# huggingface/open-muse

Measured on AMD Instinct MI355X. Metric: images/sec/node (MaskGit train step, 256^2, bs=64/GPU), higher is better.
Workload: dtype bf16 (transformer GEMM/attention operands; f32 accumulate, residual, norms, loss) + bf16x3 tokenizer (f32 activations, f32-class products as 3 bf16 MFMAs); parity of this mode was not measured in this run (a --full run measures it); 1 GPU; MaskGit train step: MaskGitVQGAN f16-256 encode (bf16x3) + cosine mask + MaskGitTransformer config B (configs/imagenet.yaml: hidden 768, 24 layers, 16 heads, vocab 2048, seq 257) fwd+bwd (bf16 MFMA, f32 accum/residual) + AdamW; global_batch=64, per_gpu_batch=64, resolution=256, seq_len=257, parallelism=dp1, vqgan_dtype=bf16x3, random_init=True, wgrad_stream=True

## Files before the change

### open-muse_amd/csrc/embed.hip

```cpp
#include <cstring>
#include <rocprim/device/device_radix_sort.hpp>
#include "common.h"
#include "../../include/muse_hip.h"

namespace emb {
constexpr int SEG = 64;

__global__ void prep_kernel(const int64_t* __restrict__ ids, unsigned* __restrict__ keys, unsigned* __restrict__ vals, int ntok, int vocab) {
  const int t = blockIdx.x * blockDim.x + threadIdx.x;
  if (t < ntok) {
    const int64_t id = ids[t];
    keys[t] = (id >= 0 && id < vocab) ? (unsigned)id : (unsigned)vocab;
    vals[t] = (unsigned)t;
  }
}

__global__ __launch_bounds__(1024) void table_kernel(const unsigned* __restrict__ keys, int ntok, int vocab, int* __restrict__ start,
                                                     int* __restrict__ segfirst) {
  __shared__ int wsum[16];
  __shared__ int carry_s;
  for (int v = threadIdx.x; v <= vocab; v += 1024) {
    int lo = 0, hi = ntok;
    while (lo < hi) { const int mid = (lo + hi) >> 1; if (keys[mid] < (unsigned)v) lo = mid + 1; else hi = mid; }
    start[v] = lo;
  }
  if (threadIdx.x == 0) carry_s = 0;
  __syncthreads();
  const int lane = threadIdx.x & 63, wave = threadIdx.x >> 6;
  for (int base = 0; base <= vocab; base += 1024) {
    const int v = base + threadIdx.x;
    int n = 0;
    if (v < vocab) n = (start[v + 1] - start[v] + SEG - 1) / SEG;
    int incl = n;
#pragma unroll
    for (int o = 1; o < 64; o <<= 1) { const int y = __shfl_up(incl, o, 64); if (lane >= o) incl += y; }
    if (lane == 63) wsum[wave] = incl;
    __syncthreads();
    int woff = 0;
    for (int w = 0; w < wave; ++w) woff += wsum[w];
    const int carry = carry_s;
    if (v <= vocab) segfirst[v] = carry + woff + incl - n;
    __syncthreads();
    if (threadIdx.x == 1023) carry_s = carry + woff + incl;
    __syncthreads();
  }
}

__global__ __launch_bounds__(256) void segment_kernel(const unsigned* __restrict__ order, const int* __restrict__ start,
                                                      const int* __restrict__ segfirst, const float* __restrict__ dout,
                                                      float* __restrict__ partial, int hidden, int vocab) {
  const int b = blockIdx.x;
  if (b >= segfirst[vocab]) return;
  int lo = 0, hi = vocab;
  while (hi - lo > 1) { const int mid = (lo + hi) >> 1; if (segfirst[mid] <= b) lo = mid; else hi = mid; }
  const int v = lo;
  const int p0 = start[v] + (b - segfirst[v]) * SEG, p1 = min(start[v + 1], p0 + SEG);
  float acc[16];
#pragma unroll
  for (int j = 0; j < 16; ++j) acc[j] = 0.f;
  const int ncol = (hidden - (int)threadIdx.x + 255) / 256;
  int h = p0;
  for (; h + 4 <= p1; h += 4) {
    const float* s0 = dout + (long)order[h] * hidden;
    const float* s1 = dout + (long)order[h + 1] * hidden;
    const float* s2 = dout + (long)order[h + 2] * hidden;
    const float* s3 = dout + (long)order[h + 3] * hidden;
#pragma unroll
    for (int j = 0; j < 16; ++j) {
      if (j < ncol) {
        const int c = threadIdx.x + j * 256;
        const float a0 = s0[c], a1 = s1[c], a2 = s2[c], a3 = s3[c];
        acc[j] = (((acc[j] + a0) + a1) + a2) + a3;
      }
    }
  }
  for (; h < p1; ++h) {
    const float* src = dout + (long)order[h] * hidden;
#pragma unroll
    for (int j = 0; j < 16; ++j) if (j < ncol) acc[j] += src[threadIdx.x + j * 256];
  }
  float* dst = partial + (long)b * hidden;
#pragma unroll
  for (int j = 0; j < 16; ++j) { const int c = threadIdx.x + j * 256; if (c < hidden) dst[c] = acc[j]; }
}

__global__ __launch_bounds__(256) void row_kernel(const int* __restrict__ segfirst, const float* __restrict__ partial,
                                                  float* __restrict__ dword, int hidden, int accumulate) {
  const int v = blockIdx.x, s0 = segfirst[v], s1 = segfirst[v + 1];
  for (int c = threadIdx.x; c < hidden; c += 256) {
    float s = 0.f;
    for (int k = s0; k < s1; ++k) s += partial[(long)k * hidden + c];
    float* d = dword + (long)v * hidden + c;
    *d = accumulate ? *d + s : s;
  }
}

__global__ void pos_kernel(const float* __restrict__ dout, float* __restrict__ dpos, int batch, int seq, int hidden, int acc) {
  const int s = blockIdx.x;
  for (int c = threadIdx.x; c < hidden; c += blockDim.x) {
    float a = 0.f;
    for (int b = 0; b < batch; ++b) a += dout[((long)b * seq + s) * hidden + c];
    float* d = dpos + (long)s * hidden + c;
    *d = acc ? *d + a : a;
  }
}

static inline size_t al(size_t x) { return (x + 255) & ~(size_t)255; }
struct Layout { size_t keys_in, keys_out, vals_in, vals_out, start, segfirst, partial, temp, temp_bytes, total; int maxseg; };
static inline int key_bits(int vocab) { int b = 1; while ((1 << b) <= vocab) ++b; return b; }
static int layout(int ntok, int hidden, int vocab, Layout& L) {
  size_t tb = 0;
  const hipError_t e = rocprim::radix_sort_pairs((void*)nullptr, tb, (const unsigned*)nullptr, (unsigned*)nullptr, (const unsigned*)nullptr,
                                                 (unsigned*)nullptr, (size_t)ntok, 0u, (unsigned)key_bits(vocab), (hipStream_t)0);
  if (e != hipSuccess) return (int)e;
  L.maxseg = vocab + ntok / SEG + 1;
  size_t o = 0;
  L.keys_in = o; o += al((size_t)ntok * 4);
  L.keys_out = o; o += al((size_t)ntok * 4);
  L.vals_in = o; o += al((size_t)ntok * 4);
  L.vals_out = o; o += al((size_t)ntok * 4);
  L.start = o; o += al((size_t)(vocab + 1) * 4);
  L.segfirst = o; o += al((size_t)(vocab + 1) * 4);
  L.partial = o; o += al((size_t)L.maxseg * hidden * 4);
  L.temp = o; L.temp_bytes = tb; o += al(tb);
  L.total = o;
  return 0;
}
}

extern "C" int64_t muse_embed_bwd2_scratch_bytes(int32_t batch, int32_t seq, int32_t hidden, int32_t vocab) {
  emb::Layout L;
  if (batch <= 0 || seq <= 0) return 0;
  if (emb::layout(batch * seq, hidden, vocab, L)) return -1;
  return (int64_t)L.total;
}

extern "C" int muse_embed_bwd2(const int64_t* ids, const float* dout, float* dword, float* dpos, void* scratch, int64_t scratch_bytes,
                               int32_t batch, int32_t seq, int32_t hidden, int32_t vocab, int32_t accumulate, void* stream) {
  if (hidden > 4096 || vocab <= 0) return MUSE_ERR_UNSUPPORTED;
  const int ntok = batch * seq;
  if (ntok <= 0) return 0;
  emb::Layout L;
  if (int e = emb::layout(ntok, hidden, vocab, L)) return e;
  if ((size_t)scratch_bytes < L.total || (((uintptr_t)scratch) & 255)) return MUSE_ERR_BAD_ARG;
  hipStream_t s = (hipStream_t)stream;
  unsigned char* base = (unsigned char*)scratch;
  unsigned* keys_in = (unsigned*)(base + L.keys_in);
  unsigned* keys_out = (unsigned*)(base + L.keys_out);
  unsigned* vals_in = (unsigned*)(base + L.vals_in);
  unsigned* vals_out = (unsigned*)(base + L.vals_out);
  int* start = (int*)(base + L.start);
  int* segfirst = (int*)(base + L.segfirst);
  float* partial = (float*)(base + L.partial);
  hipLaunchKernelGGL(emb::prep_kernel, dim3((ntok + 255) / 256), dim3(256), 0, s, ids, keys_in, vals_in, ntok, vocab);
  size_t tb = L.temp_bytes;
  const hipError_t e = rocprim::radix_sort_pairs((void*)(base + L.temp), tb, (const unsigned*)keys_in, keys_out, (const unsigned*)vals_in, vals_out,
                                                 (size_t)ntok, 0u, (unsigned)emb::key_bits(vocab), s);
  if (e != hipSuccess) return (int)e;
  hipLaunchKernelGGL(emb::table_kernel, dim3(1), dim3(1024), 0, s, (const unsigned*)keys_out, ntok, vocab, start, segfirst);
  hipLaunchKernelGGL(emb::segment_kernel, dim3(L.maxseg), dim3(256), 0, s, (const unsigned*)vals_out, (const int*)start, (const int*)segfirst,
                     dout, partial, hidden, vocab);
  hipLaunchKernelGGL(emb::row_kernel, dim3(vocab), dim3(256), 0, s, (const int*)segfirst, (const float*)partial, dword, hidden, accumulate);
  hipLaunchKernelGGL(emb::pos_kernel, dim3(seq), dim3(256), 0, s, dout, dpos, batch, seq, hidden, accumulate);
  return (int)hipGetLastError();
}
```

### open-muse_amd/csrc/rowops.hip

```cpp
#include "common.h"
#include "../../include/muse_hip.h"

template <typename TI, typename TO>
__global__ __launch_bounds__(256) void ln_fwd_kernel(const TI* __restrict__ x, const float* __restrict__ w,
                                                     const float* __restrict__ res, TO* __restrict__ y,
                                                     float* __restrict__ mean_o, float* __restrict__ rstd_o, int rows,
                                                     int cols, float eps) {
  const int lane = threadIdx.x & 63;
  const int row = blockIdx.x * 4 + (threadIdx.x >> 6);
  if (row >= rows) return;
  const TI* xr = x + (long)row * cols;
  float s = 0.f;
  for (int c = lane * 4; c < cols; c += 256) { float v[4]; V4<TI>::load(xr + c, v); s += (v[0] + v[1]) + (v[2] + v[3]); }
  const float mean = wave_sum(s) / (float)cols;
  float q = 0.f;
  for (int c = lane * 4; c < cols; c += 256) {
    float v[4]; V4<TI>::load(xr + c, v);
#pragma unroll
    for (int j = 0; j < 4; ++j) { const float d = v[j] - mean; q = fmaf(d, d, q); }
  }
  const float rstd = 1.0f / sqrtf(wave_sum(q) / (float)cols + eps);
  if (lane == 0) { mean_o[row] = mean; rstd_o[row] = rstd; }
  for (int c = lane * 4; c < cols; c += 256) {
    float v[4], g[4], o[4];
    V4<TI>::load(xr + c, v); V4<float>::load(w + c, g);
#pragma unroll
    for (int j = 0; j < 4; ++j) o[j] = (v[j] - mean) * rstd * g[j];
    if (res) { float r[4]; V4<float>::load(res + (long)row * cols + c, r);
#pragma unroll
      for (int j = 0; j < 4; ++j) o[j] += r[j]; }
    V4<TO>::store(y + (long)row * cols + c, o);
  }
}

template <typename TI, typename TO>
static int ln_fwd_launch(const void* x, const float* w, const float* res, void* y, float* mean, float* rstd, int rows,
                         int cols, float eps, hipStream_t s) {
  hipLaunchKernelGGL((ln_fwd_kernel<TI, TO>), dim3((rows + 3) / 4), dim3(256), 0, s, (const TI*)x, w, res, (TO*)y, mean, rstd,
                     rows, cols, eps);
  return (int)hipGetLastError();
}

extern "C" int muse_layernorm_fwd(const void* x, int32_t x_dtype, const float* w, const float* residual, void* y,
                                  int32_t y_dtype, float* mean, float* rstd, int32_t rows, int32_t cols, float eps,
                                  void* stream) {
  if (cols % 4 || rows <= 0) return rows == 0 ? 0 : MUSE_ERR_BAD_ARG;
  hipStream_t s = (hipStream_t)stream;
  if (x_dtype == MUSE_F32 && y_dtype == MUSE_F32) return ln_fwd_launch<float, float>(x, w, residual, y, mean, rstd, rows, cols, eps, s);
  if (x_dtype == MUSE_F32 && y_dtype == MUSE_BF16) return ln_fwd_launch<float, bf16_t>(x, w, residual, y, mean, rstd, rows, cols, eps, s);
  if (x_dtype == MUSE_BF16 && y_dtype == MUSE_F32) return ln_fwd_launch<bf16_t, float>(x, w, residual, y, mean, rstd, rows, cols, eps, s);
  if (x_dtype == MUSE_BF16 && y_dtype == MUSE_BF16) return ln_fwd_launch<bf16_t, bf16_t>(x, w, residual, y, mean, rstd, rows, cols, eps, s);
  return MUSE_ERR_BAD_ARG;
}

#define LN_BWD_ROWS 16
template <typename TDY, typename TX, typename TDX, int NIT>
__global__ __launch_bounds__(256) void ln_bwd_kernel(const TDY* __restrict__ dy, const TX* __restrict__ x,
                                                     const float* __restrict__ w, const float* __restrict__ mean,
                                                     const float* __restrict__ rstd, const float* __restrict__ dres,
                                                     TDX* __restrict__ dx, bf16_t* __restrict__ dx2, float* __restrict__ dwp, int rows,
                                                     int cols) {
  __shared__ float red[4][NIT * 256];
  const int lane = threadIdx.x & 63, wave = threadIdx.x >> 6;
  float dwacc[NIT][4];
#pragma unroll
  for (int it = 0; it < NIT; ++it)
#pragma unroll
    for (int j = 0; j < 4; ++j) dwacc[it][j] = 0.f;
  const int rbeg = blockIdx.x * LN_BWD_ROWS + wave * (LN_BWD_ROWS / 4);
#ifdef LN_BWD_PREFETCH
  constexpr bool PF = NIT <= 4;
#else
  constexpr bool PF = false;
#endif
  typename V4<TDY>::raw dn[PF ? NIT : 1];
  typename V4<TX>::raw xn[PF ? NIT : 1];
  auto fetch = [&](int row) {
#pragma unroll
    for (int it = 0; it < (PF ? NIT : 0); ++it) {
      const int c = it * 256 + lane * 4;
      if (c < cols) { dn[it] = V4<TDY>::load_raw(dy + (long)row * cols + c); xn[it] = V4<TX>::load_raw(x + (long)row * cols + c); }
    }
  };
  if (PF && rbeg < rows) fetch(rbeg);
  for (int rr = 0; rr < LN_BWD_ROWS / 4; ++rr) {
    const int row = rbeg + rr;
    if (row >= rows) break;
    const float mu = mean[row], rs = rstd[row];
    const TDY* dyr = dy + (long)row * cols;
    const TX* xr = x + (long)row * cols;
    float s1 = 0.f, s2 = 0.f;
    float gk[NIT][4], xh[NIT][4];
    typename V4<TDY>::raw dc[PF ? NIT : 1];
    typename V4<TX>::raw xc[PF ? NIT : 1];
    if constexpr (PF) {
#pragma unroll
      for (int it = 0; it < NIT; ++it) { dc[it] = dn[it]; xc[it] = xn[it]; }
      if (rr + 1 < LN_BWD_ROWS / 4 && row + 1 < rows) fetch(row + 1);
    }
#pragma unroll
    for (int it = 0; it < NIT; ++it) {
      const int c = it * 256 + lane * 4;
      if (c < cols) {
        float d[4], v[4], g[4];
        if constexpr (PF) { V4<TDY>::unpack(dc[it], d); V4<TX>::unpack(xc[it], v); }
        else { V4<TDY>::load(dyr + c, d); V4<TX>::load(xr + c, v); }
        V4<float>::load(w + c, g);
#pragma unroll
        for (int j = 0; j < 4; ++j) {
          xh[it][j] = (v[j] - mu) * rs;
          gk[it][j] = d[j] * g[j];
          s1 += gk[it][j];
          s2 = fmaf(gk[it][j], xh[it][j], s2);
          dwacc[it][j] = fmaf(d[j], xh[it][j], dwacc[it][j]);
        }
      }
    }
    const float c1 = wave_sum(s1) / (float)cols, c2 = wave_sum(s2) / (float)cols;
#pragma unroll
    for (int it = 0; it < NIT; ++it) {
      const int c = it * 256 + lane * 4;
      if (c < cols) {
// ... 547 lines not shown
        if (live) dwacc[k][j] = fmaf(d[j], xh[k][j], dwacc[k][j]);
      }
    }
    const float c1 = pair_sum(s1, red, (rr & 1) * 2, pair, wip) / (float)inter;
    const float c2 = pair_sum(s2, red, (rr & 1) * 2 + 1, pair, wip) / (float)inter;
    if (live) {
      bf16_t* dr = dab + (long)row * 2 * inter;
#pragma unroll
      for (int k = 0; k < NK; ++k) {
        float a[8], b[8], da[8], db[8];
        unpack8(ra[k], a); unpack8(rb[k], b);
#pragma unroll
        for (int j = 0; j < 8; ++j) {
          const float dh = rs * (gk[k][j] - c1 - xh[k][j] * c2);
          da[j] = dh * b[j] * gelu_erf_grad_t<true>(a[j]);
          db[j] = dh * gelu_erf_t<true>(a[j]);
        }
        *(u32x4*)(dr + k * 1024 + t * 8) = pack8(da);
        *(u32x4*)(dr + inter + k * 1024 + t * 8) = pack8(db);
      }
    }
  }
  if (r0 < rows) {
#pragma unroll
    for (int k = 0; k < NK; ++k) {
      float* o = dwp + (long)prow * inter + k * 1024 + t * 8;
      *(f32x4*)o = f32x4{dwacc[k][0], dwacc[k][1], dwacc[k][2], dwacc[k][3]};
      *(f32x4*)(o + 4) = f32x4{dwacc[k][4], dwacc[k][5], dwacc[k][6], dwacc[k][7]};
    }
  }
}

static bool ffn_mid_wide_ok(int32_t dtype, int32_t inter, int bit) {
  static const int on = []() { const char* e = getenv("MUSE_FFN_MID_WIDE"); return e ? atoi(e) : 1; }();
  return ((on >> bit) & 1) && dtype == MUSE_BF16 && inter % 1024 == 0 && inter <= 4096;
}

extern "C" int muse_ffn_mid_rows_per_block(void) { return FFN_ROWS; }

extern "C" int muse_ffn_mid_fwd(const void* ab, const float* w, void* h, void* hm, float* mean, float* rstd, int32_t dtype,
                                int32_t rows, int32_t inter, float eps, void* stream) {
  if (inter % 4 || inter > 4096) return MUSE_ERR_UNSUPPORTED;
  if (rows <= 0) return 0;
  hipStream_t s = (hipStream_t)stream;
  const dim3 grid((rows + FFN_ROWS - 1) / FFN_ROWS);
  const int nv = (inter + 1023) / 1024;
  if (ffn_mid_wide_ok(dtype, inter, 0) && !((((uintptr_t)ab) | ((uintptr_t)h) | ((uintptr_t)hm) | ((uintptr_t)w)) & 15)) {
    const dim3 g2((grid.x + 1) / 2);
#define FF2(NK) hipLaunchKernelGGL((ffn_mid_fwd2_kernel<NK>), g2, dim3(256), 0, s, (const bf16_t*)ab, w, (bf16_t*)h, (bf16_t*)hm, mean, rstd, rows, eps)
    if (nv == 1) FF2(1); else if (nv == 2) FF2(2); else if (nv == 3) FF2(3); else FF2(4);
#undef FF2
    return (int)hipGetLastError();
  }
#define FF(T, NV) hipLaunchKernelGGL((ffn_mid_fwd_kernel<T, NV>), grid, dim3(256), 0, s, (const T*)ab, w, (T*)h, (T*)hm, mean, rstd, rows, inter, eps)
  if (dtype == MUSE_F32) { if (nv == 1) FF(float, 1); else if (nv == 2) FF(float, 2); else if (nv == 3) FF(float, 3); else FF(float, 4); }
  else { if (nv == 1) FF(bf16_t, 1); else if (nv == 2) FF(bf16_t, 2); else if (nv == 3) FF(bf16_t, 3); else FF(bf16_t, 4); }
#undef FF
  return (int)hipGetLastError();
}

extern "C" int muse_ffn_mid_bwd(const void* dhm, const void* h, const void* ab, const float* w, const float* mean,
                                const float* rstd, void* dab, float* dw_partial, int32_t dtype, int32_t rows, int32_t inter,
                                void* stream) {
  if (inter % 4 || inter > 4096) return MUSE_ERR_UNSUPPORTED;
  if (rows <= 0) return 0;
  hipStream_t s = (hipStream_t)stream;
  const dim3 grid((rows + FFN_ROWS - 1) / FFN_ROWS);
  const int nv = (inter + 1023) / 1024;
  if (h && ffn_mid_wide_ok(dtype, inter, 1) && !((((uintptr_t)dhm) | ((uintptr_t)h) | ((uintptr_t)ab) | ((uintptr_t)dab) | ((uintptr_t)w) | ((uintptr_t)dw_partial)) & 15)) {
    const dim3 g2((grid.x + 1) / 2);
#define FB2(NK) hipLaunchKernelGGL((ffn_mid_bwd2_kernel<NK>), g2, dim3(256), 0, s, (const bf16_t*)dhm, (const bf16_t*)h, (const bf16_t*)ab, w, mean, rstd, (bf16_t*)dab, dw_partial, rows)
    if (nv == 1) FB2(1); else if (nv == 2) FB2(2); else if (nv == 3) FB2(3); else FB2(4);
#undef FB2
    return (int)hipGetLastError();
  }
#define FB(T, NV) do { if (h) hipLaunchKernelGGL((ffn_mid_bwd_kernel<T, NV, false>), grid, dim3(256), 0, s, (const T*)dhm, (const T*)h, (const T*)ab, w, mean, rstd, (T*)dab, dw_partial, rows, inter); \
                       else hipLaunchKernelGGL((ffn_mid_bwd_kernel<T, NV, true>), grid, dim3(256), 0, s, (const T*)dhm, (const T*)nullptr, (const T*)ab, w, mean, rstd, (T*)dab, dw_partial, rows, inter); } while (0)
  if (dtype == MUSE_F32) { if (nv == 1) FB(float, 1); else if (nv == 2) FB(float, 2); else if (nv == 3) FB(float, 3); else FB(float, 4); }
  else { if (nv == 1) FB(bf16_t, 1); else if (nv == 2) FB(bf16_t, 2); else if (nv == 3) FB(bf16_t, 3); else FB(bf16_t, 4); }
#undef FB
  return (int)hipGetLastError();
}

__global__ __launch_bounds__(1024) void colsum_kernel(const float* __restrict__ in, float* __restrict__ out, int rows, int cols, int acc) {
  __shared__ float red[64][17];
  const int c16 = threadIdx.x & 15, rg = threadIdx.x >> 4;
  const int c = blockIdx.x * 16 + c16;
  float s0 = 0.f, s1 = 0.f;
  if (c < cols) {
    int r = rg;
    for (; r + 64 < rows; r += 128) { s0 += in[(long)r * cols + c]; s1 += in[(long)(r + 64) * cols + c]; }
    if (r < rows) s0 += in[(long)r * cols + c];
  }
  red[rg][c16] = s0 + s1;
  __syncthreads();
  if (rg == 0 && c < cols) {
    float s = 0.f;
#pragma unroll
    for (int k = 0; k < 64; ++k) s += red[k][c16];
    out[c] = acc ? out[c] + s : s;
  }
}
extern "C" int muse_colsum(const float* in, float* out, int32_t rows, int32_t cols, int32_t accumulate, void* stream) {
  if (cols <= 0) return 0;
  hipLaunchKernelGGL(colsum_kernel, dim3((cols + 15) / 16), dim3(1024), 0, (hipStream_t)stream, in, out, rows, cols, accumulate);
  return (int)hipGetLastError();
}

__global__ __launch_bounds__(256) void add_rowvec_kernel(float* __restrict__ x, const float* __restrict__ b, long n, int cols) {
  for (long i = (long)blockIdx.x * 256 + threadIdx.x; i < n; i += (long)gridDim.x * 256) x[i] += b[i % cols];
}
extern "C" int muse_add_rowvec(float* x, const float* b, int64_t rows, int32_t cols, void* stream) {
  if (rows <= 0 || cols <= 0) return 0;
  const long n = (long)rows * cols;
  hipLaunchKernelGGL(add_rowvec_kernel, dim3((unsigned)((n + 255) / 256 > 4096 ? 4096 : (n + 255) / 256)), dim3(256), 0, (hipStream_t)stream, x, b, n, cols);
  return (int)hipGetLastError();
}

constexpr int kBiasGradRows = 128;
template <typename T>
__global__ __launch_bounds__(256) void bias_grad_partial_kernel(const T* __restrict__ dy, float* __restrict__ part, long rows, int cols, long ld) {
  const int c = blockIdx.x * 256 + threadIdx.x;
  if (c >= cols) return;
  const long r0 = (long)blockIdx.y * kBiasGradRows;
  const long r1 = r0 + kBiasGradRows < rows ? r0 + kBiasGradRows : rows;
  float s = 0.f;
  for (long r = r0; r < r1; ++r) s += Elem<T>::load(dy + r * ld + c);
  part[(long)blockIdx.y * cols + c] = s;
}
extern "C" int muse_bias_grad_rows_per_block(void) { return kBiasGradRows; }
extern "C" int muse_bias_grad_partial(const void* dy, int32_t dtype, float* partial, int64_t rows, int32_t cols, int64_t ld, void* stream) {
  if (rows <= 0 || cols <= 0) return 0;
  if (dtype != MUSE_F32 && dtype != MUSE_BF16) return MUSE_ERR_BAD_ARG;
  const dim3 grid((cols + 255) / 256, (unsigned)((rows + kBiasGradRows - 1) / kBiasGradRows));
  if (dtype == MUSE_F32) hipLaunchKernelGGL((bias_grad_partial_kernel<float>), grid, dim3(256), 0, (hipStream_t)stream, (const float*)dy, partial, (long)rows, cols, (long)ld);
  else hipLaunchKernelGGL((bias_grad_partial_kernel<bf16_t>), grid, dim3(256), 0, (hipStream_t)stream, (const bf16_t*)dy, partial, (long)rows, cols, (long)ld);
  return (int)hipGetLastError();
}

template <typename T>
__global__ __launch_bounds__(256) void softmax_fwd_kernel(const T* __restrict__ x, T* __restrict__ y, long rows, int cols, long ld) {
  const int lane = threadIdx.x & 63;
  const long row = (long)blockIdx.x * 4 + (threadIdx.x >> 6);
  if (row >= rows) return;
  const T* xr = x + row * ld;
  T* yr = y + row * ld;
  float m = -INFINITY;
  for (int c = lane; c < cols; c += 64) m = fmaxf(m, Elem<T>::load(xr + c));
  m = wave_max(m);
  float s = 0.f;
  for (int c = lane; c < cols; c += 64) s += expf(Elem<T>::load(xr + c) - m);
  s = wave_sum(s);
  const float inv = 1.0f / s;
  for (int c = lane; c < (int)ld; c += 64) {
    const float v = c < cols ? expf(Elem<T>::load(xr + c) - m) * inv : 0.f;
    Elem<T>::store(yr + c, v);
  }
}
extern "C" int muse_softmax_fwd(const void* x, void* y, int32_t dtype, int64_t rows, int32_t cols, int64_t ld, void* stream) {
  if (rows <= 0) return 0;
  dim3 grid((unsigned)((rows + 3) / 4));
  if (dtype == MUSE_F32) hipLaunchKernelGGL(softmax_fwd_kernel<float>, grid, dim3(256), 0, (hipStream_t)stream, (const float*)x, (float*)y, (long)rows, cols, (long)ld);
  else hipLaunchKernelGGL(softmax_fwd_kernel<bf16_t>, grid, dim3(256), 0, (hipStream_t)stream, (const bf16_t*)x, (bf16_t*)y, (long)rows, cols, (long)ld);
  return (int)hipGetLastError();
}

template <typename T>
__global__ __launch_bounds__(256) void softmax_bwd_kernel(const T* __restrict__ p, const T* __restrict__ dp, T* __restrict__ ds,
                                                          long rows, int cols, long ld) {
  const int lane = threadIdx.x & 63;
  const long row = (long)blockIdx.x * 4 + (threadIdx.x >> 6);
  if (row >= rows) return;
  const T* pr = p + row * ld;
  const T* dr = dp + row * ld;
  T* sr = ds + row * ld;
  float s = 0.f;
  for (int c = lane; c < cols; c += 64) s = fmaf(Elem<T>::load(pr + c), Elem<T>::load(dr + c), s);
  s = wave_sum(s);
  for (int c = lane; c < (int)ld; c += 64) {
    const float v = c < cols ? Elem<T>::load(pr + c) * (Elem<T>::load(dr + c) - s) : 0.f;
    Elem<T>::store(sr + c, v);
  }
}
extern "C" int muse_softmax_bwd(const void* p, const void* dp, void* ds, int32_t dtype, int64_t rows, int32_t cols,
                                int64_t ld, void* stream) {
  if (rows <= 0) return 0;
  dim3 grid((unsigned)((rows + 3) / 4));
  if (dtype == MUSE_F32) hipLaunchKernelGGL(softmax_bwd_kernel<float>, grid, dim3(256), 0, (hipStream_t)stream, (const float*)p, (const float*)dp, (float*)ds, (long)rows, cols, (long)ld);
// ... 264 lines not shown
    for (; h + 4 <= n; h += 4) {
      const float* s0 = dout + (long)hits[h] * hidden;
      const float* s1 = dout + (long)hits[h + 1] * hidden;
      const float* s2 = dout + (long)hits[h + 2] * hidden;
      const float* s3 = dout + (long)hits[h + 3] * hidden;
#pragma unroll
      for (int j = 0; j < 16; ++j) {
        if (j < ncol) {
          const int c = threadIdx.x + j * 256;
          const float a0 = s0[c], a1 = s1[c], a2 = s2[c], a3 = s3[c];
          acc[j] = (((acc[j] + a0) + a1) + a2) + a3;
        }
      }
    }
    for (; h < n; ++h) {
      const float* src = dout + (long)hits[h] * hidden;
#pragma unroll
      for (int j = 0; j < 16; ++j) if (j < ncol) acc[j] += src[threadIdx.x + j * 256];
    }
    __syncthreads();
  }
  float* dst = partial + ((long)sp * vocab + v) * hidden;
#pragma unroll
  for (int j = 0; j < 16; ++j) { const int c = threadIdx.x + j * 256; if (c < hidden) dst[c] = acc[j]; }
}
__global__ void embed_bwd_reduce_kernel(const float* __restrict__ partial, float* __restrict__ dword, long n, int acc, int nsplit) {
  for (long i = (long)blockIdx.x * blockDim.x + threadIdx.x; i < n; i += (long)gridDim.x * blockDim.x) {
    float s = 0.f;
    for (int sp = 0; sp < nsplit; ++sp) s += partial[(long)sp * n + i];
    dword[i] = acc ? dword[i] + s : s;
  }
}
__global__ void embed_bwd_pos_kernel(const float* __restrict__ dout, float* __restrict__ dpos, int batch, int seq, int hidden, int acc) {
  const int s = blockIdx.x;
  for (int c = threadIdx.x; c < hidden; c += blockDim.x) {
    float a = 0.f;
    for (int b = 0; b < batch; ++b) a += dout[((long)b * seq + s) * hidden + c];
    float* d = dpos + (long)s * hidden + c;
    *d = acc ? *d + a : a;
  }
}
extern "C" int muse_embed_bwd(const int64_t* ids, const float* dout, float* dword, float* dpos, float* scratch,
                              int32_t batch, int32_t seq, int32_t hidden, int32_t vocab, int32_t accumulate, void* stream) {
  if (hidden > 4096) return MUSE_ERR_UNSUPPORTED;
  if (batch * seq <= 0) return 0;
  hipStream_t s = (hipStream_t)stream;
  const int nsplit = emb_splits(hidden, vocab);
  hipLaunchKernelGGL(embed_bwd_partial_kernel, dim3(vocab, nsplit), dim3(256), 0, s, ids, dout, scratch, batch * seq, hidden, vocab, nsplit);
  const long n = (long)vocab * hidden;
  hipLaunchKernelGGL(embed_bwd_reduce_kernel, dim3(ew_grid(n)), dim3(256), 0, s, (const float*)scratch, dword, n, accumulate, nsplit);
  hipLaunchKernelGGL(embed_bwd_pos_kernel, dim3(seq), dim3(256), 0, s, dout, dpos, batch, seq, hidden, accumulate);
  return (int)hipGetLastError();
}
extern "C" int64_t muse_embed_bwd_scratch_floats(int32_t hidden, int32_t vocab) { return (int64_t)emb_splits(hidden, vocab) * vocab * hidden; }

template <typename T>
__global__ __launch_bounds__(256) void ce_fwd_kernel(const T* __restrict__ logits, const int64_t* __restrict__ labels,
                                                     float* __restrict__ row_loss, float* __restrict__ lse_o, long rows,
                                                     int vocab, long ld, float ls) {
  const int lane = threadIdx.x & 63;
  const long row = (long)blockIdx.x * 4 + (threadIdx.x >> 6);
  if (row >= rows) return;
  const T* xr = logits + row * ld;
  float m = -INFINITY, sx = 0.f;
  for (int c = lane; c < vocab; c += 64) { const float v = Elem<T>::load(xr + c); m = fmaxf(m, v); sx += v; }
  m = wave_max(m);
  float s = 0.f;
  for (int c = lane; c < vocab; c += 64) s += expf(Elem<T>::load(xr + c) - m);
  s = wave_sum(s);
  sx = wave_sum(sx);
  const float lse = m + logf(s);
  if (lane == 0) {
    lse_o[row] = lse;
    const int64_t lab = labels[row];
    float l = 0.f;
    if (lab >= 0 && lab < vocab) {
      const float nll = lse - Elem<T>::load(xr + lab);
      const float smooth = lse - sx / (float)vocab;
      l = (1.0f - ls) * nll + ls * smooth;
    }
    row_loss[row] = l;
  }
}
__global__ __launch_bounds__(1024) void ce_reduce_kernel(const float* __restrict__ row_loss, const int64_t* __restrict__ labels,
                                                         float* __restrict__ out, long rows, int vocab) {
  __shared__ double ssum[16];
  __shared__ int scnt[16];
  double s = 0.0; int n = 0;
  for (long r = threadIdx.x; r < rows; r += 1024) {
    const int64_t lab = labels[r];
    if (lab >= 0 && lab < vocab) { s += (double)row_loss[r]; ++n; }
  }
  s = wave_sum_d(s);
#pragma unroll
  for (int o = 32; o > 0; o >>= 1) n += __shfl_xor(n, o, 64);
  if ((threadIdx.x & 63) == 0) { ssum[threadIdx.x >> 6] = s; scnt[threadIdx.x >> 6] = n; }
  __syncthreads();
  if (threadIdx.x == 0) {
    double t = 0.0; int c = 0;
    for (int i = 0; i < 16; ++i) { t += ssum[i]; c += scnt[i]; }
    out[0] = (float)(t / (double)c);
    out[1] = (float)c;
  }
}
extern "C" int muse_cross_entropy_fwd(const void* logits, int32_t dtype, const int64_t* labels, float* row_loss, float* lse,
                                      float* loss_out, int64_t rows, int32_t vocab, int64_t ld, float label_smoothing,
                                      void* stream) {
  if (rows <= 0) return MUSE_ERR_BAD_ARG;
  hipStream_t s = (hipStream_t)stream;
  dim3 grid((unsigned)((rows + 3) / 4));
  if (dtype == MUSE_F32) hipLaunchKernelGGL(ce_fwd_kernel<float>, grid, dim3(256), 0, s, (const float*)logits, labels, row_loss, lse, (long)rows, vocab, (long)ld, label_smoothing);
  else hipLaunchKernelGGL(ce_fwd_kernel<bf16_t>, grid, dim3(256), 0, s, (const bf16_t*)logits, labels, row_loss, lse, (long)rows, vocab, (long)ld, label_smoothing);
  hipLaunchKernelGGL(ce_reduce_kernel, dim3(1), dim3(1024), 0, s, (const float*)row_loss, labels, loss_out, (long)rows, vocab);
  return (int)hipGetLastError();
}

template <typename T, typename TO>
__global__ __launch_bounds__(256) void ce_bwd_kernel(const T* __restrict__ logits, const int64_t* __restrict__ labels,
                                                     const float* __restrict__ lse, const float* __restrict__ loss_out,
                                                     const float* __restrict__ gout, TO* __restrict__ dl, long rows, int vocab,
                                                     long ld, float ls) {
  const int lane = threadIdx.x & 63;
  const long row = (long)blockIdx.x * 4 + (threadIdx.x >> 6);
  if (row >= rows) return;
  const int64_t lab = labels[row];
  TO* dr = dl + row * ld;
  if (lab < 0 || lab >= vocab) {
    for (int c = lane; c < (int)ld; c += 64) Elem<TO>::store(dr + c, 0.f);
    return;
  }
  const float g = gout[0] / loss_out[1];
  const float l = lse[row];
  const T* xr = logits + row * ld;
  const float off = ls / (float)vocab;
  for (int c = lane; c < (int)ld; c += 64) {
    float p = 0.f;
    if (c < vocab) {
      p = expf(Elem<T>::load(xr + c) - l) - off;
      if (c == (int)lab) p -= (1.0f - ls);
    }
    Elem<TO>::store(dr + c, p * g);
  }
}
extern "C" int muse_cross_entropy_bwd(const void* logits, int32_t dtype, const int64_t* labels, const float* lse,
                                      const float* loss_out, const float* grad_out, void* dlogits, int32_t dl_dtype,
                                      int64_t rows, int32_t vocab, int64_t ld, float label_smoothing, void* stream) {
  if (rows <= 0) return 0;
  hipStream_t s = (hipStream_t)stream;
  dim3 grid((unsigned)((rows + 3) / 4));
#define CEB(T, TO) hipLaunchKernelGGL((ce_bwd_kernel<T, TO>), grid, dim3(256), 0, s, (const T*)logits, labels, lse, loss_out, grad_out, (TO*)dlogits, (long)rows, vocab, (long)ld, label_smoothing)
  if (dtype == MUSE_F32 && dl_dtype == MUSE_F32) CEB(float, float);
  else if (dtype == MUSE_F32 && dl_dtype == MUSE_BF16) CEB(float, bf16_t);
  else if (dtype == MUSE_BF16 && dl_dtype == MUSE_F32) CEB(bf16_t, float);
  else CEB(bf16_t, bf16_t);
#undef CEB
  return (int)hipGetLastError();
}

__device__ __forceinline__ bool soft_row_active(long row, int S1, const int64_t* labels, long& srow) {
  const long b = row / S1;
  const int s = (int)(row - b * S1);
  srow = b * (S1 - 1) + s - 1;
  return s >= 1 && labels[row] != -100;
}

template <int NCH, bool VEC>
__device__ __forceinline__ void soft_row_load(const float* __restrict__ xr, const float* __restrict__ pr, int lane, float (&x)[NCH * 4],
                                              float (&p)[NCH * 4]) {
  if constexpr (VEC) {
#pragma unroll
    for (int j = 0; j < NCH; ++j) {
      const int c = (j * 64 + lane) * 4;
      const f32x4 a = *(const f32x4*)(xr + c), q = *(const f32x4*)(pr + c);
#pragma unroll
      for (int e = 0; e < 4; ++e) { x[j * 4 + e] = a[e]; p[j * 4 + e] = q[e]; }
    }
  } else {
#pragma unroll
    for (int i = 0; i < NCH * 4; ++i) { x[i] = xr[i * 64 + lane]; p[i] = pr[i * 64 + lane]; }
  }
}

template <int NCH, bool VEC>
__global__ __launch_bounds__(256) void soft_ce_fwd_kernel(const float* __restrict__ logits, const int64_t* __restrict__ labels,
                                                          const float* __restrict__ soft, float* __restrict__ row_loss,
                                                          float* __restrict__ lse_o, float* __restrict__ psum_o, long rows, int S1,
                                                          int K, long ld) {
  const int lane = threadIdx.x & 63;
  const long row = (long)blockIdx.x * 4 + (threadIdx.x >> 6);
  if (row >= rows) return;
  long srow;
  if (!soft_row_active(row, S1, labels, srow)) {
    if (lane == 0) { row_loss[row] = 0.f; lse_o[row] = 0.f; psum_o[row] = 0.f; }
    return;
// ... 230 lines not shown
      if ((threadIdx.x & 63) == 0) atomicAdd(stats + 1, und);
    }
  }
}
extern "C" int muse_cast_f32_to_f16(const float* in, void* out, int64_t n, float scale, int32_t* stats, void* stream) {
  if (n <= 0) return 0;
  if ((((uintptr_t)in) & 15) || (((uintptr_t)out) & 7)) return MUSE_ERR_ALIGN;
  hipLaunchKernelGGL(cast_f2h_kernel, dim3(ew_grid((n + 3) / 4)), dim3(256), 0, (hipStream_t)stream, in, (_Float16*)out, (long)n, scale, (int*)stats);
  return (int)hipGetLastError();
}
extern "C" int muse_cast_bf16_to_f32(const void* in, float* out, int64_t n, void* stream) {
  if (n <= 0) return 0;
  if ((((uintptr_t)out) & 15) || (((uintptr_t)in) & 7)) return MUSE_ERR_ALIGN;
  hipLaunchKernelGGL(cast_b2f_kernel, dim3(ew_grid((n + 3) / 4)), dim3(256), 0, (hipStream_t)stream, (const bf16_t*)in, out, (long)n);
  return (int)hipGetLastError();
}

__global__ __launch_bounds__(256) void mask_sample_kernel(const int64_t* __restrict__ tokens, const int64_t* __restrict__ class_ids,
                                                          const float* __restrict__ timesteps, const float* __restrict__ noise,
                                                          int64_t* __restrict__ input_ids, int64_t* __restrict__ labels,
                                                          float* __restrict__ mask_prob, int seq, int64_t mask_id,
                                                          int64_t codebook, float min_rate) {
  __shared__ float nz[1024];
  __shared__ int perm[1024];
  const int b = blockIdx.x;
  for (int i = threadIdx.x; i < seq; i += 256) nz[i] = noise[(long)b * seq + i];
  __syncthreads();
  const float arg = (timesteps[b] * 3.14159265358979323846f) * 0.5f;
  float prob = (float)cos((double)arg);
  prob = fmaxf(prob, min_rate);
  float kf = rintf((float)seq * prob);
  kf = fmaxf(kf, 1.0f);
  const int k = (int)kf;
  for (int i = threadIdx.x; i < seq; i += 256) {
    const float v = nz[i];
    int r = 0;
    for (int j = 0; j < seq; ++j) { const float u = nz[j]; r += (u < v) || (u == v && j < i); }
    perm[r] = i;
  }
  __syncthreads();
  int64_t* ir = input_ids + (long)b * (seq + 1);
  int64_t* lr = labels + (long)b * (seq + 1);
  if (threadIdx.x == 0) { ir[0] = class_ids[b] + codebook; lr[0] = -100; mask_prob[b] = prob; }
  for (int j = threadIdx.x; j < seq; j += 256) {
    const bool masked = perm[j] < k;
    const int64_t t = tokens[(long)b * seq + j];
    ir[j + 1] = masked ? mask_id : t;
    lr[j + 1] = masked ? t : (int64_t)-100;
  }
}
extern "C" int muse_mask_sample(const int64_t* tokens, const int64_t* class_ids, const float* timesteps, const float* noise,
                                int64_t* input_ids, int64_t* labels, float* mask_prob, int32_t batch, int32_t seq,
                                int64_t mask_id, int64_t codebook_size, float min_masking_rate, void* stream) {
  if (seq > 1024 || seq <= 0) return MUSE_ERR_UNSUPPORTED;
  if (batch <= 0) return 0;
  hipLaunchKernelGGL(mask_sample_kernel, dim3(batch), dim3(256), 0, (hipStream_t)stream, tokens, class_ids, timesteps, noise,
                     input_ids, labels, mask_prob, seq, mask_id, codebook_size, min_masking_rate);
  return (int)hipGetLastError();
}

__global__ void sum_slices_kernel(const float* __restrict__ ws, float* __restrict__ out, int ns, long n, long stride, int acc) {
  const long n4 = n >> 2;
  for (long i = (long)blockIdx.x * blockDim.x + threadIdx.x; i < n4; i += (long)gridDim.x * blockDim.x) {
    float a[4] = {0.f, 0.f, 0.f, 0.f};
    if (acc) V4<float>::load(out + i * 4, a);
    for (int s = 0; s < ns; ++s) {
      float t[4]; V4<float>::load(ws + s * stride + i * 4, t);
#pragma unroll
      for (int j = 0; j < 4; ++j) a[j] += t[j];
    }
    V4<float>::store(out + i * 4, a);
  }
}
extern "C" int muse_sum_slices(const float* ws, float* out, int32_t nslices, int64_t n, int64_t stride, int32_t accumulate,
                               void* stream) {
  if (n <= 0) return 0;
  if ((n & 3) || (stride & 3) || (((uintptr_t)ws) & 15) || (((uintptr_t)out) & 15)) return MUSE_ERR_ALIGN;
  hipLaunchKernelGGL(sum_slices_kernel, dim3(ew_grid(n / 4)), dim3(256), 0, (hipStream_t)stream, ws, out, nslices, (long)n,
                     (long)stride, accumulate);
  return (int)hipGetLastError();
}

#define MUSE_SUM_MAX_JOBS 16
struct SumJob { const float* ws; float* out; long n, stride; int ns, acc, first_item, kind; };
struct SumJobs { SumJob j[MUSE_SUM_MAX_JOBS]; int n; };
__global__ __launch_bounds__(1024) void sum_multi_kernel(const SumJobs J) {
  __shared__ float red[64][17];
  int k = 0;
#pragma unroll
  for (int i = 1; i < MUSE_SUM_MAX_JOBS; ++i) k += (i < J.n && (int)blockIdx.x >= J.j[i].first_item) ? 1 : 0;
  const SumJob jb = J.j[k];
  const int item = (int)blockIdx.x - jb.first_item;
  if (jb.kind == 0) {
    const long i = (long)item * 4096 + threadIdx.x * 4;
    if (i < jb.n) {
      float a[4] = {0.f, 0.f, 0.f, 0.f};
      if (jb.acc) V4<float>::load(jb.out + i, a);
      for (int s = 0; s < jb.ns; ++s) {
        float t[4]; V4<float>::load(jb.ws + s * jb.stride + i, t);
#pragma unroll
        for (int q = 0; q < 4; ++q) a[q] += t[q];
      }
      V4<float>::store(jb.out + i, a);
    }
    return;
  }
  const int c16 = threadIdx.x & 15, rg = threadIdx.x >> 4;
  const int cols = (int)jb.n, rows = jb.ns;
  const int c = item * 16 + c16;
  float s0 = 0.f, s1 = 0.f;
  if (c < cols) {
    int r = rg;
    for (; r + 64 < rows; r += 128) { s0 += jb.ws[(long)r * cols + c]; s1 += jb.ws[(long)(r + 64) * cols + c]; }
    if (r < rows) s0 += jb.ws[(long)r * cols + c];
  }
  red[rg][c16] = s0 + s1;
  __syncthreads();
  if (rg == 0 && c < cols) {
    float sum = 0.f;
#pragma unroll
    for (int q = 0; q < 64; ++q) sum += red[q][c16];
    jb.out[c] = jb.acc ? jb.out[c] + sum : sum;
  }
}
extern "C" int muse_sum_multi(const void* const* ws, void* const* out, const int32_t* nslices, const int64_t* n, const int64_t* stride,
                              const int32_t* accumulate, const int32_t* kind, int32_t njobs, void* stream) {
  if (njobs <= 0) return 0;
  if (njobs > MUSE_SUM_MAX_JOBS) return MUSE_ERR_BAD_ARG;
  SumJobs J;
  int items = 0;
  for (int i = 0; i < njobs; ++i) {
    if (n[i] <= 0 || nslices[i] < 1 || (kind[i] != 0 && kind[i] != 1)) return MUSE_ERR_BAD_ARG;
    if (kind[i] == 0 && ((n[i] & 3) || (stride[i] & 3) || (((uintptr_t)ws[i]) & 15) || (((uintptr_t)out[i]) & 15))) return MUSE_ERR_ALIGN;
    SumJob& j = J.j[i];
    j.ws = (const float*)ws[i]; j.out = (float*)out[i]; j.n = n[i]; j.stride = stride[i]; j.ns = nslices[i]; j.acc = accumulate[i];
    j.first_item = items; j.kind = kind[i];
    items += kind[i] == 0 ? (int)((n[i] / 4 + 1023) / 1024) : (int)((n[i] + 15) / 16);
  }
  for (int i = njobs; i < MUSE_SUM_MAX_JOBS; ++i) J.j[i] = J.j[0];
  J.n = njobs;
  hipLaunchKernelGGL(sum_multi_kernel, dim3(items), dim3(1024), 0, (hipStream_t)stream, J);
  return (int)hipGetLastError();
}

template <typename TO>
__global__ __launch_bounds__(256) void sum_slices_epi_kernel(const float* __restrict__ ws, int ns, long stride, const float* __restrict__ bias,
                                                            const TO* __restrict__ residual, long ldr, TO* __restrict__ out, long ldc,
                                                            long rows, int cols) {
  const int vpr = cols >> 2;
  const long n = rows * vpr;
  for (long i = (long)blockIdx.x * 256 + threadIdx.x; i < n; i += (long)gridDim.x * 256) {
    const long r = i / vpr;
    const int c = (int)(i - r * vpr) * 4;
    float a[4] = {0.f, 0.f, 0.f, 0.f};
    for (int k = 0; k < ns; ++k) {
      float t[4]; V4<float>::load(ws + k * stride + r * cols + c, t);
#pragma unroll
      for (int q = 0; q < 4; ++q) a[q] += t[q];
    }
    if (bias) { float b[4]; V4<float>::load(bias + c, b);
#pragma unroll
      for (int q = 0; q < 4; ++q) a[q] += b[q]; }
    if (residual) { float t[4]; V4<TO>::load(residual + r * ldr + c, t);
#pragma unroll
      for (int q = 0; q < 4; ++q) a[q] += t[q]; }
    V4<TO>::store(out + r * ldc + c, a);
  }
}
extern "C" int muse_sum_slices_epilogue(const float* ws, int32_t nslices, int64_t stride, const float* bias, const void* residual, int64_t ldr,
                                        void* out, int32_t out_dtype, int64_t ldc, int64_t rows, int32_t cols, void* stream) {
  if (rows <= 0 || cols <= 0) return 0;
  if ((cols & 3) || (stride & 3) || (ldc & 3) || (ldr & 3) || nslices < 1) return MUSE_ERR_BAD_ARG;
  const int ob = out_dtype == MUSE_BF16 ? 7 : 15;
  if ((((uintptr_t)ws) & 15) || (((uintptr_t)bias) & 15) || (((uintptr_t)out) & ob) || (((uintptr_t)residual) & ob)) return MUSE_ERR_ALIGN;
  const long n = rows * (cols >> 2);
  const dim3 grid(ew_grid(n));
  if (out_dtype == MUSE_BF16)
    hipLaunchKernelGGL(sum_slices_epi_kernel<bf16_t>, grid, dim3(256), 0, (hipStream_t)stream, ws, nslices, (long)stride, bias, (const bf16_t*)residual,
                       (long)ldr, (bf16_t*)out, (long)ldc, (long)rows, cols);
  else
    hipLaunchKernelGGL(sum_slices_epi_kernel<float>, grid, dim3(256), 0, (hipStream_t)stream, ws, nslices, (long)stride, bias, (const float*)residual,
                       (long)ldr, (float*)out, (long)ldc, (long)rows, cols);
  return (int)hipGetLastError();
}

extern "C" int muse_version(void) { return 1; }
```

Baseline: 1251 images/s.

## Vectorize and batch loads in embed, layernorm, CE, colsum and slice-sum kernels

Several reduction kernels now keep more loads in flight and use wider loads. The embedding row and position sums use float4 loads with 16 reads issued before accumulating. Layernorm forward gets a register-resident variant for up to 1024 columns, and cross-entropy forward gets one that holds the whole 2048-vocab row in registers. Column-sum and sum-multi now handle 32 columns per block with float4 loads, 8 rows in flight and a waves-per-EU hint. The aim is to hide memory latency in small bandwidth-bound kernels, at the cost of more registers and code specialization.

```diff
diff --git a/open-muse_amd/csrc/embed.hip b/open-muse_amd/csrc/embed.hip
--- a/open-muse_amd/csrc/embed.hip
+++ b/open-muse_amd/csrc/embed.hip
@@ -84,25 +84,53 @@
   for (int j = 0; j < 16; ++j) { const int c = threadIdx.x + j * 256; if (c < hidden) dst[c] = acc[j]; }
 }
 
+constexpr int FLY = 16;
+template <int W> __device__ __forceinline__ void ldw(const float* p, float (&v)[W]);
+template <> __device__ __forceinline__ void ldw<4>(const float* p, float (&v)[4]) { V4<float>::load(p, v); }
+template <> __device__ __forceinline__ void ldw<1>(const float* p, float (&v)[1]) { v[0] = *p; }
+template <int W> __device__ __forceinline__ void stw(float* p, const float (&v)[W]);
+template <> __device__ __forceinline__ void stw<4>(float* p, const float (&v)[4]) { V4<float>::store(p, v); }
+template <> __device__ __forceinline__ void stw<1>(float* p, const float (&v)[1]) { *p = v[0]; }
+
+template <int W>
+__device__ __forceinline__ void chain_sum(const float* __restrict__ src, long stride, int n, float* __restrict__ dst, int accumulate) {
+  float s[W];
+#pragma unroll
+  for (int j = 0; j < W; ++j) s[j] = 0.f;
+  for (int k = 0; k < n; k += FLY) {
+    float t[FLY][W];
+#pragma unroll
+    for (int u = 0; u < FLY; ++u) if (k + u < n) ldw<W>(src + (long)(k + u) * stride, t[u]);
+#pragma unroll
+    for (int u = 0; u < FLY; ++u) {
+      if (k + u < n) {
+#pragma unroll
+        for (int j = 0; j < W; ++j) s[j] += t[u][j];
+      }
+    }
+  }
+  if (accumulate) {
+    float o[W];
+    ldw<W>(dst, o);
+#pragma unroll
+    for (int j = 0; j < W; ++j) s[j] = o[j] + s[j];
+  }
+  stw<W>(dst, s);
+}
+
+template <int W>
 __global__ __launch_bounds__(256) void row_kernel(const int* __restrict__ segfirst, const float* __restrict__ partial,
                                                   float* __restrict__ dword, int hidden, int accumulate) {
   const int v = blockIdx.x, s0 = segfirst[v], s1 = segfirst[v + 1];
-  for (int c = threadIdx.x; c < hidden; c += 256) {
-    float s = 0.f;
-    for (int k = s0; k < s1; ++k) s += partial[(long)k * hidden + c];
-    float* d = dword + (long)v * hidden + c;
-    *d = accumulate ? *d + s : s;
-  }
-}
-
-__global__ void pos_kernel(const float* __restrict__ dout, float* __restrict__ dpos, int batch, int seq, int hidden, int acc) {
+  for (int c = threadIdx.x * W; c < hidden; c += 256 * W)
+    chain_sum<W>(partial + (long)s0 * hidden + c, hidden, s1 - s0, dword + (long)v * hidden + c, accumulate);
+}
+
+template <int W>
+__global__ __launch_bounds__(256) void pos_kernel(const float* __restrict__ dout, float* __restrict__ dpos, int batch, int seq, int hidden, int acc) {
   const int s = blockIdx.x;
-  for (int c = threadIdx.x; c < hidden; c += blockDim.x) {
-    float a = 0.f;
-    for (int b = 0; b < batch; ++b) a += dout[((long)b * seq + s) * hidden + c];
-    float* d = dpos + (long)s * hidden + c;
-    *d = acc ? *d + a : a;
-  }
+  for (int c = threadIdx.x * W; c < hidden; c += 256 * W)
+    chain_sum<W>(dout + (long)s * hidden + c, (long)seq * hidden, batch, dpos + (long)s * hidden + c, acc);
 }
 
 static inline size_t al(size_t x) { return (x + 255) & ~(size_t)255; }
@@ -160,7 +188,13 @@
   hipLaunchKernelGGL(emb::table_kernel, dim3(1), dim3(1024), 0, s, (const unsigned*)keys_out, ntok, vocab, start, segfirst);
   hipLaunchKernelGGL(emb::segment_kernel, dim3(L.maxseg), dim3(256), 0, s, (const unsigned*)vals_out, (const int*)start, (const int*)segfirst,
                      dout, partial, hidden, vocab);
-  hipLaunchKernelGGL(emb::row_kernel, dim3(vocab), dim3(256), 0, s, (const int*)segfirst, (const float*)partial, dword, hidden, accumulate);
-  hipLaunchKernelGGL(emb::pos_kernel, dim3(seq), dim3(256), 0, s, dout, dpos, batch, seq, hidden, accumulate);
+  if (!(hidden & 3) && !(((uintptr_t)dword) & 15))
+    hipLaunchKernelGGL(emb::row_kernel<4>, dim3(vocab), dim3(256), 0, s, (const int*)segfirst, (const float*)partial, dword, hidden, accumulate);
+  else
+    hipLaunchKernelGGL(emb::row_kernel<1>, dim3(vocab), dim3(256), 0, s, (const int*)segfirst, (const float*)partial, dword, hidden, accumulate);
+  if (!(hidden & 3) && !((((uintptr_t)dout) | ((uintptr_t)dpos)) & 15))
+    hipLaunchKernelGGL(emb::pos_kernel<4>, dim3(seq), dim3(256), 0, s, dout, dpos, batch, seq, hidden, accumulate);
+  else
+    hipLaunchKernelGGL(emb::pos_kernel<1>, dim3(seq), dim3(256), 0, s, dout, dpos, batch, seq, hidden, accumulate);
   return (int)hipGetLastError();
 }
diff --git a/open-muse_amd/csrc/rowops.hip b/open-muse_amd/csrc/rowops.hip
--- a/open-muse_amd/csrc/rowops.hip
+++ b/open-muse_amd/csrc/rowops.hip
@@ -33,11 +33,56 @@
   }
 }
 
+template <typename TI, typename TO, int NV>
+__global__ __launch_bounds__(256) void ln_fwd_reg_kernel(const TI* __restrict__ x, const float* __restrict__ w,
+                                                         const float* __restrict__ res, TO* __restrict__ y,
+                                                         float* __restrict__ mean_o, float* __restrict__ rstd_o, int rows,
+                                                         int cols, float eps) {
+  const int lane = threadIdx.x & 63;
+  const int row = blockIdx.x * 4 + (threadIdx.x >> 6);
+  if (row >= rows) return;
+  const TI* xr = x + (long)row * cols;
+  float v[NV][4];
+#pragma unroll
+  for (int i = 0; i < NV; ++i) { const int c = lane * 4 + i * 256; if (c < cols) V4<TI>::load(xr + c, v[i]); }
+  float s = 0.f;
+#pragma unroll
+  for (int i = 0; i < NV; ++i) if (lane * 4 + i * 256 < cols) s += (v[i][0] + v[i][1]) + (v[i][2] + v[i][3]);
+  const float mean = wave_sum(s) / (float)cols;
+  float q = 0.f;
+#pragma unroll
+  for (int i = 0; i < NV; ++i) {
+    if (lane * 4 + i * 256 < cols) {
+#pragma unroll
+      for (int j = 0; j < 4; ++j) { const float d = v[i][j] - mean; q = fmaf(d, d, q); }
+    }
+  }
+  const float rstd = 1.0f / sqrtf(wave_sum(q) / (float)cols + eps);
+  if (lane == 0) { mean_o[row] = mean; rstd_o[row] = rstd; }
+#pragma unroll
+  for (int i = 0; i < NV; ++i) {
+    const int c = lane * 4 + i * 256;
+    if (c < cols) {
+      float g[4], o[4];
+      V4<float>::load(w + c, g);
+#pragma unroll
+      for (int j = 0; j < 4; ++j) o[j] = (v[i][j] - mean) * rstd * g[j];
+      if (res) { float r[4]; V4<float>::load(res + (long)row * cols + c, r);
+#pragma unroll
+        for (int j = 0; j < 4; ++j) o[j] += r[j]; }
+      V4<TO>::store(y + (long)row * cols + c, o);
+    }
+  }
+}
+
 template <typename TI, typename TO>
 static int ln_fwd_launch(const void* x, const float* w, const float* res, void* y, float* mean, float* rstd, int rows,
                          int cols, float eps, hipStream_t s) {
-  hipLaunchKernelGGL((ln_fwd_kernel<TI, TO>), dim3((rows + 3) / 4), dim3(256), 0, s, (const TI*)x, w, res, (TO*)y, mean, rstd,
-                     rows, cols, eps);
+  const dim3 grid((rows + 3) / 4);
+#define LNF(NV) hipLaunchKernelGGL((ln_fwd_reg_kernel<TI, TO, NV>), grid, dim3(256), 0, s, (const TI*)x, w, res, (TO*)y, mean, rstd, rows, cols, eps)
+  if (cols <= 256) LNF(1); else if (cols <= 512) LNF(2); else if (cols <= 768) LNF(3); else if (cols <= 1024) LNF(4);
+  else hipLaunchKernelGGL((ln_fwd_kernel<TI, TO>), grid, dim3(256), 0, s, (const TI*)x, w, res, (TO*)y, mean, rstd, rows, cols, eps);
+#undef LNF
   return (int)hipGetLastError();
 }
 
@@ -751,28 +796,69 @@
   return (int)hipGetLastError();
 }
 
-__global__ __launch_bounds__(1024) void colsum_kernel(const float* __restrict__ in, float* __restrict__ out, int rows, int cols, int acc) {
-  __shared__ float red[64][17];
-  const int c16 = threadIdx.x & 15, rg = threadIdx.x >> 4;
-  const int c = blockIdx.x * 16 + c16;
-  float s0 = 0.f, s1 = 0.f;
+constexpr int CS_COLS = 32;
+constexpr int CS_THREADS = 1024;
+constexpr int CS_FLY = 8;
+constexpr int CS_FLY_SCALAR = 3;
+
+template <bool VEC>
+__device__ __forceinline__ void colsum_load4(const float* __restrict__ row, int c, int cols, float (&v)[4]) {
+  if (VEC) {
+    V4<float>::load(row + c, v);
+  } else {
+#pragma unroll
+    for (int j = 0; j < 4; ++j) if (c + j < cols) v[j] = row[c + j];
+  }
+}
+
+template <bool VEC>
+__device__ __forceinline__ void colsum_item(const float* __restrict__ in, float* __restrict__ out, int rows, int cols, int acc, int item,
+                                            float (*red)[64][CS_COLS + 1]) {
+  const int q4 = threadIdx.x & 7, chain = (threadIdx.x >> 3) & 1, rg = threadIdx.x >> 4;
+  const int c = item * CS_COLS + q4 * 4;
+  float s[4] = {0.f, 0.f, 0.f, 0.f};
+  constexpr int FLY = VEC ? CS_FLY : CS_FLY_SCALAR;
   if (c < cols) {
-    int r = rg;
-    for (; r + 64 < rows; r += 128) { s0 += in[(long)r * cols + c]; s1 += in[(long)(r + 64) * cols + c]; }
-    if (r < rows) s0 += in[(long)r * cols + c];
-  }
-  red[rg][c16] = s0 + s1;
+    for (int r = rg + 64 * chain; r < rows; r += 128 * FLY) {
+      float a[FLY][4];
+#pragma unroll
+      for (int k = 0; k < FLY; ++k) {
+#pragma unroll
+        for (int j = 0; j < 4; ++j) a[k][j] = 0.f;
+        if (r + 128 * k < rows) colsum_load4<VEC>(in + (long)(r + 128 * k) * cols, c, cols, a[k]);
+      }
+#pragma unroll
+      for (int k = 0; k < FLY; ++k) {
+        if (r + 128 * k < rows) {
+#pragma unroll
+          for (int j = 0; j < 4; ++j) s[j] += a[k][j];
+        }
+      }
+    }
+  }
+#pragma unroll
+  for (int j = 0; j < 4; ++j) red[chain][rg][q4 * 4 + j] = s[j];
   __syncthreads();
-  if (rg == 0 && c < cols) {
-    float s = 0.f;
-#pragma unroll
-    for (int k = 0; k < 64; ++k) s += red[k][c16];
-    out[c] = acc ? out[c] + s : s;
-  }
+  const int co = item * CS_COLS + (int)threadIdx.x;
+  if (threadIdx.x < CS_COLS && co < cols) {
+    float t = 0.f;
+#pragma unroll
+    for (int k = 0; k < 64; ++k) t += red[0][k][threadIdx.x] + red[1][k][threadIdx.x];
+    out[co] = acc ? out[co] + t : t;
+  }
+}
+static inline bool colsum_vec_ok(const float* in, long cols) { return !(cols & 3) && !(((uintptr_t)in) & 15); }
+
+template <bool VEC>
+__global__ __launch_bounds__(CS_THREADS) __attribute__((amdgpu_waves_per_eu(8, 8))) void colsum_kernel(const float* __restrict__ in, float* __restrict__ out, int rows, int cols, int acc) {
+  __shared__ float red[2][64][CS_COLS + 1];
+  colsum_item<VEC>(in, out, rows, cols, acc, (int)blockIdx.x, red);
 }
 extern "C" int muse_colsum(const float* in, float* out, int32_t rows, int32_t cols, int32_t accumulate, void* stream) {
   if (cols <= 0) return 0;
-  hipLaunchKernelGGL(colsum_kernel, dim3((cols + 15) / 16), dim3(1024), 0, (hipStream_t)stream, in, out, rows, cols, accumulate);
+  const dim3 grid((cols + CS_COLS - 1) / CS_COLS);
+  if (colsum_vec_ok(in, cols)) hipLaunchKernelGGL(colsum_kernel<true>, grid, dim3(CS_THREADS), 0, (hipStream_t)stream, in, out, rows, cols, accumulate);
+  else hipLaunchKernelGGL(colsum_kernel<false>, grid, dim3(CS_THREADS), 0, (hipStream_t)stream, in, out, rows, cols, accumulate);
   return (int)hipGetLastError();
 }
 
@@ -1203,6 +1289,40 @@
     row_loss[row] = l;
   }
 }
+constexpr int CE_REG = 32;
+template <typename T>
+__global__ __launch_bounds__(256) void ce_fwd_reg_kernel(const T* __restrict__ logits, const int64_t* __restrict__ labels,
+                                                         float* __restrict__ row_loss, float* __restrict__ lse_o, long rows,
+                                                         int vocab, long ld, float ls) {
+  const int lane = threadIdx.x & 63;
+  const long row = (long)blockIdx.x * 4 + (threadIdx.x >> 6);
+  if (row >= rows) return;
+  const T* xr = logits + row * ld;
+  float x[CE_REG];
+#pragma unroll
+  for (int k = 0; k < CE_REG; ++k) { const int c = lane + 64 * k; if (c < vocab) x[k] = Elem<T>::load(xr + c); }
+  float m = -INFINITY, sx = 0.f;
+#pragma unroll
+  for (int k = 0; k < CE_REG; ++k) if (lane + 64 * k < vocab) { m = fmaxf(m, x[k]); sx += x[k]; }
+  m = wave_max(m);
+  float s = 0.f;
+#pragma unroll
+  for (int k = 0; k < CE_REG; ++k) if (lane + 64 * k < vocab) s += expf(x[k] - m);
+  s = wave_sum(s);
+  sx = wave_sum(sx);
+  const float lse = m + logf(s);
+  if (lane == 0) {
+    lse_o[row] = lse;
+    const int64_t lab = labels[row];
+    float l = 0.f;
+    if (lab >= 0 && lab < vocab) {
+      const float nll = lse - Elem<T>::load(xr + lab);
+      const float smooth = lse - sx / (float)vocab;
+      l = (1.0f - ls) * nll + ls * smooth;
+    }
+    row_loss[row] = l;
+  }
+}
 __global__ __launch_bounds__(1024) void ce_reduce_kernel(const float* __restrict__ row_loss, const int64_t* __restrict__ labels,
                                                          float* __restrict__ out, long rows, int vocab) {
   __shared__ double ssum[16];
@@ -1230,7 +1350,11 @@
   if (rows <= 0) return MUSE_ERR_BAD_ARG;
   hipStream_t s = (hipStream_t)stream;
   dim3 grid((unsigned)((rows + 3) / 4));
-  if (dtype == MUSE_F32) hipLaunchKernelGGL(ce_fwd_kernel<float>, grid, dim3(256), 0, s, (const float*)logits, labels, row_loss, lse, (long)rows, vocab, (long)ld, label_smoothing);
+  if (vocab <= 64 * CE_REG) {
+    if (dtype == MUSE_F32) hipLaunchKernelGGL(ce_fwd_reg_kernel<float>, grid, dim3(256), 0, s, (const float*)logits, labels, row_loss, lse, (long)rows, vocab, (long)ld, label_smoothing);
+    else hipLaunchKernelGGL(ce_fwd_reg_kernel<bf16_t>, grid, dim3(256), 0, s, (const bf16_t*)logits, labels, row_loss, lse, (long)rows, vocab, (long)ld, label_smoothing);
+  }
+  else if (dtype == MUSE_F32) hipLaunchKernelGGL(ce_fwd_kernel<float>, grid, dim3(256), 0, s, (const float*)logits, labels, row_loss, lse, (long)rows, vocab, (long)ld, label_smoothing);
   else hipLaunchKernelGGL(ce_fwd_kernel<bf16_t>, grid, dim3(256), 0, s, (const bf16_t*)logits, labels, row_loss, lse, (long)rows, vocab, (long)ld, label_smoothing);
   hipLaunchKernelGGL(ce_reduce_kernel, dim3(1), dim3(1024), 0, s, (const float*)row_loss, labels, loss_out, (long)rows, vocab);
   return (int)hipGetLastError();
@@ -1627,46 +1751,39 @@
 }
 
 #define MUSE_SUM_MAX_JOBS 16
-struct SumJob { const float* ws; float* out; long n, stride; int ns, acc, first_item, kind; };
+constexpr int SUM_SLICE_ITEM = CS_THREADS * 4;
+struct SumJob { const float* ws; float* out; long n, stride; int ns, acc, first_item, kind, vec; };
 struct SumJobs { SumJob j[MUSE_SUM_MAX_JOBS]; int n; };
-__global__ __launch_bounds__(1024) void sum_multi_kernel(const SumJobs J) {
-  __shared__ float red[64][17];
+__global__ __launch_bounds__(CS_THREADS) __attribute__((amdgpu_waves_per_eu(8, 8))) void sum_multi_kernel(const SumJobs J) {
+  __shared__ float red[2][64][CS_COLS + 1];
   int k = 0;
 #pragma unroll
   for (int i = 1; i < MUSE_SUM_MAX_JOBS; ++i) k += (i < J.n && (int)blockIdx.x >= J.j[i].first_item) ? 1 : 0;
   const SumJob jb = J.j[k];
   const int item = (int)blockIdx.x - jb.first_item;
   if (jb.kind == 0) {
-    const long i = (long)item * 4096 + threadIdx.x * 4;
+    const long i = (long)item * SUM_SLICE_ITEM + threadIdx.x * 4;
     if (i < jb.n) {
       float a[4] = {0.f, 0.f, 0.f, 0.f};
       if (jb.acc) V4<float>::load(jb.out + i, a);
-      for (int s = 0; s < jb.ns; ++s) {
-        float t[4]; V4<float>::load(jb.ws + s * jb.stride + i, t);
-#pragma unroll
-        for (int q = 0; q < 4; ++q) a[q] += t[q];
+      for (int s = 0; s < jb.ns; s += 8) {
+        float t[8][4];
+#pragma unroll
+        for (int u = 0; u < 8; ++u) if (s + u < jb.ns) V4<float>::load(jb.ws + (s + u) * jb.stride + i, t[u]);
+#pragma unroll
+        for (int u = 0; u < 8; ++u) {
+          if (s + u < jb.ns) {
+#pragma unroll
+            for (int q = 0; q < 4; ++q) a[q] += t[u][q];
+          }
+        }
       }
       V4<float>::store(jb.out + i, a);
     }
     return;
   }
-  const int c16 = threadIdx.x & 15, rg = threadIdx.x >> 4;
-  const int cols = (int)jb.n, rows = jb.ns;
-  const int c = item * 16 + c16;
-  float s0 = 0.f, s1 = 0.f;
-  if (c < cols) {
-    int r = rg;
-    for (; r + 64 < rows; r += 128) { s0 += jb.ws[(long)r * cols + c]; s1 += jb.ws[(long)(r + 64) * cols + c]; }
-    if (r < rows) s0 += jb.ws[(long)r * cols + c];
-  }
-  red[rg][c16] = s0 + s1;
-  __syncthreads();
-  if (rg == 0 && c < cols) {
-    float sum = 0.f;
-#pragma unroll
-    for (int q = 0; q < 64; ++q) sum += red[q][c16];
-    jb.out[c] = jb.acc ? jb.out[c] + sum : sum;
-  }
+  if (jb.vec) colsum_item<true>(jb.ws, jb.out, jb.ns, (int)jb.n, jb.acc, item, red);
+  else colsum_item<false>(jb.ws, jb.out, jb.ns, (int)jb.n, jb.acc, item, red);
 }
 extern "C" int muse_sum_multi(const void* const* ws, void* const* out, const int32_t* nslices, const int64_t* n, const int64_t* stride,
                               const int32_t* accumulate, const int32_t* kind, int32_t njobs, void* stream) {
@@ -1679,12 +1796,12 @@
     if (kind[i] == 0 && ((n[i] & 3) || (stride[i] & 3) || (((uintptr_t)ws[i]) & 15) || (((uintptr_t)out[i]) & 15))) return MUSE_ERR_ALIGN;
     SumJob& j = J.j[i];
     j.ws = (const float*)ws[i]; j.out = (float*)out[i]; j.n = n[i]; j.stride = stride[i]; j.ns = nslices[i]; j.acc = accumulate[i];
-    j.first_item = items; j.kind = kind[i];
-    items += kind[i] == 0 ? (int)((n[i] / 4 + 1023) / 1024) : (int)((n[i] + 15) / 16);
+    j.first_item = items; j.kind = kind[i]; j.vec = kind[i] == 1 && colsum_vec_ok(j.ws, n[i]);
+    items += kind[i] == 0 ? (int)((n[i] + SUM_SLICE_ITEM - 1) / SUM_SLICE_ITEM) : (int)((n[i] + CS_COLS - 1) / CS_COLS);
   }
   for (int i = njobs; i < MUSE_SUM_MAX_JOBS; ++i) J.j[i] = J.j[0];
   J.n = njobs;
-  hipLaunchKernelGGL(sum_multi_kernel, dim3(items), dim3(1024), 0, (hipStream_t)stream, J);
+  hipLaunchKernelGGL(sum_multi_kernel, dim3(items), dim3(CS_THREADS), 0, (hipStream_t)stream, J);
   return (int)hipGetLastError();
 }
 
```

After: 1254 images/s (median of 6 runs). No clear change (+0.3%).
